# ltdoanh2004/MotionDiffusion-MoE

Hardware: AMD Instinct MI355X
Metric: denoising-steps/sec (B=32, T=196, 263-d, 8 experts) (higher is better)
Workload: dtype bf16

## Files before the change

### motiondiffusion-moe_amd/csrc/rowwise.hip

```cpp
#include "kernels.h"
#include "row.h"

namespace mdm {
extern int g_bf16_variant;
namespace {

template <int NE, bool VEC, int FMT>
__device__ __forceinline__ void ln_chain_rows(const float* __restrict__ x, bool x_h, int64_t M, int D, const float* w1,
                                              const float* b1, void* y1, int y1_h, const float* w2, const float* b2,
                                              void* y2, int y2_h) {
  const int lane = threadIdx.x & 63;
  Row<NE, VEC> ww1, bb1, ww2, bb2;
  ww1.load(w1, D, lane), bb1.load(b1, D, lane);
  if (w2) ww2.load(w2, D, lane), bb2.load(b2, D, lane);
  for (int64_t row = 2 * (blockIdx.x * (int64_t)WPB + (threadIdx.x >> 6)); row < M; row += 2 * (int64_t)gridDim.x * WPB) {
    const bool two = row + 1 < M;
    Row<NE, VEC> r, q;
    if (x_h) {
      r.template load_h16<FMT>((const uint16_t*)x + row * D, D, lane);
      q.template load_h16<FMT>((const uint16_t*)x + (two ? row + 1 : row) * D, D, lane);
    } else {
      r.load(x + row * D, D, lane);
      q.load(x + (two ? row + 1 : row) * D, D, lane);
    }
    r.layernorm(ww1, bb1, D, lane);
    q.layernorm(ww1, bb1, D, lane);
    if (y1) {
      r.template store_mode<FMT>(y1, row, D, lane, y1_h);
      if (two) q.template store_mode<FMT>(y1, row + 1, D, lane, y1_h);
    }
    if (w2) {
      r.layernorm(ww2, bb2, D, lane);
      q.layernorm(ww2, bb2, D, lane);
      r.template store_mode<FMT>(y2, row, D, lane, y2_h);
      if (two) q.template store_mode<FMT>(y2, row + 1, D, lane, y2_h);
    }
  }
}
template <int NE, bool VEC>
__global__ __launch_bounds__(256) void ln_chain_kernel(const float* __restrict__ x, int x_bf, int64_t M, int D,
                                                       const float* w1, const float* b1, void* y1, int y1_bf,
                                                       const float* w2, const float* b2, void* y2, int y2_bf) {
  const int m1 = y1_bf == 4 ? 2 : (y1_bf != 0), m2 = y2_bf == 4 ? 2 : (y2_bf != 0);
  if (((x_bf | y1_bf | y2_bf) & 3) == 2) {
    ln_chain_rows<NE, VEC, 2>(x, x_bf != 0, M, D, w1, b1, y1, m1, w2, b2, y2, m2);
  } else {
    ln_chain_rows<NE, VEC, 1>(x, x_bf != 0, M, D, w1, b1, y1, m1, w2, b2, y2, m2);
  }
}

template <int NE, bool VEC, int FMT>
__device__ __forceinline__ void style_in_rows(const float* __restrict__ x, int64_t M, int D, int S, const float* pw,
                                              const float* pb, const float* sw, const float* sb,
                                              const float* __restrict__ sc, const int* __restrict__ pos4, bool x_h,
                                              void* __restrict__ out, bool out_h) {
  const int lane = threadIdx.x & 63;
  Row<NE, VEC> pww, pbb, sww, sbb;
  if (pw) pww.load(pw, D, lane), pbb.load(pb, D, lane);
  sww.load(sw, D, lane), sbb.load(sb, D, lane);
  for (int64_t row = blockIdx.x * (int64_t)WPB + (threadIdx.x >> 6); row < M; row += (int64_t)gridDim.x * WPB) {
    const float* scb = sc + (row / S) * 2 * (int64_t)D;
    Row<NE, VEC> r, scale, shift;
    scale.load(scb, D, lane);
    shift.load(scb + D, D, lane);
    if (pos4) {
      const int p0 = pos4[row * 4 + 0], p1 = pos4[row * 4 + 1], p2 = pos4[row * 4 + 2], p3 = pos4[row * 4 + 3];
      Row<NE, VEC> a, b, c, d;
      if (x_h) {
        const uint16_t* xh = (const uint16_t*)x;
        a.template load_h16<FMT>(xh + (int64_t)p0 * D, D, lane);
        b.template load_h16<FMT>(xh + (int64_t)p1 * D, D, lane);
        c.template load_h16<FMT>(xh + (int64_t)p2 * D, D, lane);
        d.template load_h16<FMT>(xh + (int64_t)p3 * D, D, lane);
      } else {
        a.load(x + (int64_t)p0 * D, D, lane);
        b.load(x + (int64_t)p1 * D, D, lane);
        c.load(x + (int64_t)p2 * D, D, lane);
        d.load(x + (int64_t)p3 * D, D, lane);
      }
#pragma unroll
      for (int j = 0; j < NE; ++j) r.e[j] = ((a.e[j] + b.e[j]) + (c.e[j] + d.e[j])) * 0.5f;
    } else {
      if (x_h) {
        r.template load_h16<FMT>((const uint16_t*)x + row * D, D, lane);
      } else {
        r.load(x + row * D, D, lane);
      }
    }
    if (pw) {
      r.layernorm(pww, pbb, D, lane);
      float s = 0.f;
#pragma unroll
      for (int j = 0; j < NE; ++j) s += r.e[j] * r.e[j];
      const float inv = sqrtf((float)D) / fmaxf(sqrtf(wave_sum(s)), 1e-12f);
#pragma unroll
      for (int j = 0; j < NE; ++j) r.e[j] *= inv;
    }
    r.layernorm(sww, sbb, D, lane);
#pragma unroll
    for (int j = 0; j < NE; ++j) r.e[j] = silu(r.e[j] * (1.f + scale.e[j]) + shift.e[j]);
    r.template store_to<FMT>(out, row, D, lane, out_h);
  }
}
template <int NE, bool VEC>
__global__ __launch_bounds__(256) void style_in_kernel(const float* __restrict__ x, int64_t M, int D, int S,
                                                       const float* pw, const float* pb,
                                                       const float* sw, const float* sb,
                                                       const float* __restrict__ sc,
                                                       const int* __restrict__ pos4,
                                                       int x_bf,
                                                       void* __restrict__ out, int out_bf) {
  if ((x_bf | out_bf) == 2) {
    style_in_rows<NE, VEC, 2>(x, M, D, S, pw, pb, sw, sb, sc, pos4, x_bf != 0, out, out_bf != 0);
  } else {
    style_in_rows<NE, VEC, 1>(x, M, D, S, pw, pb, sw, sb, sc, pos4, x_bf != 0, out, out_bf != 0);
  }
}

template <int NE, bool VEC>
__global__ __launch_bounds__(256) void moe_gate_kernel(const float* __restrict__ x, int64_t M, int D, int E,
                                                       MoeGateParams p) {
  __shared__ int s_hist[32];
  __shared__ float s_usage[32], s_imp[32];
  if (threadIdx.x < 32) s_hist[threadIdx.x] = 0, s_usage[threadIdx.x] = 0.f, s_imp[threadIdx.x] = 0.f;
  __syncthreads();
  const int lane = threadIdx.x & 63;
  for (int64_t row = blockIdx.x * (int64_t)WPB + (threadIdx.x >> 6); row < M; row += (int64_t)gridDim.x * WPB) {
    Row<NE, VEC> xr;
    xr.load(x + row * D, D, lane);
#pragma unroll
    for (int br = 0; br < 2; ++br) {
      Row<NE, VEC> r = xr;
      r.layernorm(p.ln_w[br], p.ln_b[br], D, lane);
      r.store_as(p.hn, (int64_t)br * M + row, D, lane, p.hn_bf16);
      float logit[16];
      float mx = -INFINITY;
#pragma unroll
      for (int e = 0; e < 16; ++e) {
        logit[e] = -INFINITY;
        if (e < E) {
          Row<NE, VEC> g;
          g.load(p.gate_w[br] + (int64_t)e * D, D, lane);
          float s = 0.f;
#pragma unroll
          for (int j = 0; j < NE; ++j) s += r.e[j] * g.e[j];
          logit[e] = wave_sum(s) + p.gate_b[br][e];
          mx = fmaxf(mx, logit[e]);
        }
      }
      float den = 0.f;
#pragma unroll
      for (int e = 0; e < 16; ++e) {
        logit[e] = e < E ? expf(logit[e] - mx) : 0.f;
        den += logit[e];
      }
      int i1 = 0, i2 = 1;
      float v1 = -1.f, v2 = -1.f;
      if (p.forced_idx) {
        i1 = min(max(p.forced_idx[((int64_t)br * M + row) * 2 + 0], 0), E - 1);
        i2 = min(max(p.forced_idx[((int64_t)br * M + row) * 2 + 1], 0), E - 1);
        v1 = v2 = 0.f;
#pragma unroll
        for (int e = 0; e < 16; ++e) {
          const float pe = logit[e] / den;
          v1 = e == i1 ? pe : v1;
          v2 = e == i2 ? pe : v2;
        }
      } else {
#pragma unroll
        for (int e = 0; e < 16; ++e) {
          const float pe = logit[e] / den;
          if (e < E) {
            if (pe > v1) {
              v2 = v1, i2 = i1;
              v1 = pe, i1 = e;
            } else if (pe > v2) {
              v2 = pe, i2 = e;
            }
          }
        }
        if (!(v2 >= 0.f)) {
          i2 = i1 == 0 ? 1 : 0;
          v1 = v2 = __int_as_float(0x7fc00000);
        }
      }
      if (lane == 0) {
        const int64_t o = ((int64_t)br * M + row) * 2;
        p.top_idx[o] = i1, p.top_idx[o + 1] = i2;
        p.top_val[o] = v1, p.top_val[o + 1] = v2;
        atomicAdd(&s_hist[br * E + i1], 1);
        atomicAdd(&s_hist[br * E + i2], 1);
        atomicAdd(&s_usage[br * E + i1], 1.f);
        atomicAdd(&s_imp[br * E + i1], v1);
        atomicAdd(&s_imp[br * E + i2], v2);
      }
    }
  }
  __syncthreads();
  if (threadIdx.x < 2 * E) {
    const int g = threadIdx.x;
    p.hist[blockIdx.x * 32 + g] = s_hist[g];
    p.uimp[blockIdx.x * 64 + g] = s_usage[g];
    p.uimp[blockIdx.x * 64 + 32 + g] = s_imp[g];
  }
}

template <int NV, bool FAST, int EX = 0, int HNF = -1>
__global__ __launch_bounds__(256) void moe_gate16_kernel(const float* __restrict__ x, int64_t M, int D_rt, int E_rt,
                                                         MoeGateParams p) {
  const int E = EX > 0 ? EX : E_rt;
  const int hnf = HNF >= 0 ? HNF : p.hn_bf16;
  constexpr int D = 64 * NV;
  extern __shared__ __attribute__((aligned(16))) float gsm[];
  float* gw = gsm;
  float* lnw = gsm + 2 * E * D;
  float* lnb = lnw + 2 * D;
  int* s_hist = (int*)(lnb + 2 * D);
  float* s_usage = (float*)(s_hist + 32);
  float* s_imp = s_usage + 32;
  const int l16 = threadIdx.x & 15;
  const int64_t tpb = 16;
  const int64_t stride = (int64_t)gridDim.x * tpb;
  auto load_x = [&](int64_t base, f32x4(&r)[NV]) {
    const int64_t row = base + (threadIdx.x >> 4);
    const int64_t rc = row < M ? row : M - 1;
#pragma unroll
    for (int c = 0; c < NV; ++c) r[c] = *(const f32x4*)(x + rc * D + 4 * (l16 + 16 * c));
  };
  f32x4 vn[NV];
  if constexpr (NV <= 8)
    if (blockIdx.x * tpb < M) load_x(blockIdx.x * tpb, vn);
#pragma unroll
  for (int br = 0; br < 2; ++br) {
    const float* src = p.gate_w[br];
    const int n4 = E * D / 4;
    for (int i0 = threadIdx.x; i0 < n4; i0 += 4 * 256) {
      f32x4 t[4];
#pragma unroll
      for (int j = 0; j < 4; ++j)
        if (i0 + 256 * j < n4) t[j] = *(const f32x4*)(src + 4 * (i0 + 256 * j));
#pragma unroll
      for (int j = 0; j < 4; ++j)
        if (i0 + 256 * j < n4) *(f32x4*)(gw + br * E * D + 4 * (i0 + 256 * j)) = t[j];
    }
  }
  for (int i = threadIdx.x; i < D / 4; i += 256) {
    const f32x4 w0 = *(const f32x4*)(p.ln_w[0] + 4 * i), w1 = *(const f32x4*)(p.ln_w[1] + 4 * i);
    const f32x4 b0 = *(const f32x4*)(p.ln_b[0] + 4 * i), b1 = *(const f32x4*)(p.ln_b[1] + 4 * i);
    *(f32x4*)(lnw + 4 * i) = w0, *(f32x4*)(lnw + D + 4 * i) = w1;
    *(f32x4*)(lnb + 4 * i) = b0, *(f32x4*)(lnb + D + 4 * i) = b1;
  }
  if (threadIdx.x < 32) s_hist[threadIdx.x] = 0, s_usage[threadIdx.x] = 0.f, s_imp[threadIdx.x] = 0.f;
  __syncthreads();
  for (int64_t base = blockIdx.x * tpb; base < M; base += stride) {
    const int64_t row = base + (threadIdx.x >> 4);
    const bool ok = row < M;
    const int64_t rc = ok ? row : M - 1;
    if constexpr (NV > 8) load_x(base, vn);
    f32x4 v[NV];
    float s = 0.f;
#pragma unroll
    for (int c = 0; c < NV; ++c) {
      v[c] = vn[c];
      s += v[c][0] + v[c][1] + v[c][2] + v[c][3];
    }
    if constexpr (NV <= 8)
      if (base + stride < M) load_x(base + stride, vn);
    const float mean = group_sum<16>(s) / D;
    float q = 0.f;
#pragma unroll
    for (int c = 0; c < NV; ++c) {
      v[c] = (f32x4){v[c][0] - mean, v[c][1] - mean, v[c][2] - mean, v[c][3] - mean};
      q += v[c][0] * v[c][0] + v[c][1] * v[c][1] + v[c][2] * v[c][2] + v[c][3] * v[c][3];
    }
    const float rstd = rsqrtf(group_sum<16>(q) / D + 1e-5f);
#pragma unroll
    for (int br = 0; br < 2; ++br) {
      float logit[16];
#pragma unroll
      for (int e = 0; e < 16; ++e) logit[e] = 0.f;
      float amax = 0.f;
#pragma unroll
      for (int c = 0; c < NV; ++c) {
        const int k = 4 * (l16 + 16 * c);
        const f32x4 w = *(const f32x4*)(lnw + br * D + k), b = *(const f32x4*)(lnb + br * D + k);
        const f32x4 h = {v[c][0] * rstd * w[0] + b[0], v[c][1] * rstd * w[1] + b[1], v[c][2] * rstd * w[2] + b[2],
                         v[c][3] * rstd * w[3] + b[3]};
        amax = fmaxf(amax, fmaxf(fmaxf(fabsf(h[0]), fabsf(h[1])), fmaxf(fabsf(h[2]), fabsf(h[3]))));
        if constexpr (HNF >= 0) {
          if constexpr (HNF == 1 || HNF == 2) {
            *(uint2*)((uint16_t*)p.hn + ((int64_t)br * M + rc) * D + k) = make_uint2(pack_h16(HNF, h[0], h[1]), pack_h16(HNF, h[2], h[3]));
          } else if constexpr (HNF == 0) {
            *(f32x4*)((float*)p.hn + ((int64_t)br * M + rc) * D + k) = h;
          } else if constexpr (HNF == 4) {
            static_assert(D % 32 == 0, "lane pairs of store_x2_4p hold k and k ^ 4 of one 32-column block");
            store_x2_4p((uint16_t*)p.hn + ((int64_t)br * M + rc) * 2 * D, k, h[0], h[1], h[2], h[3]);
          }
        } else if (ok && p.hn_bf16 != 3) {
          if (p.hn_bf16 == 4) {
            store_x2_4((uint16_t*)p.hn + ((int64_t)br * M + row) * 2 * D, k, h[0], h[1], h[2], h[3]);
          } else if (p.hn_bf16 == 2) {
            *(uint2*)((uint16_t*)p.hn + ((int64_t)br * M + row) * D + k) = make_uint2(pack_h16(2, h[0], h[1]), pack_h16(2, h[2], h[3]));
          } else if (p.hn_bf16) {
            *(uint2*)((uint16_t*)p.hn + ((int64_t)br * M + row) * D + k) = make_uint2(pack_h16(1, h[0], h[1]), pack_h16(1, h[2], h[3]));
          } else {
            *(f32x4*)((float*)p.hn + ((int64_t)br * M + row) * D + k) = h;
          }
        }
#pragma unroll
        for (int e = 0; e < 16; ++e)
          if (e < E) {
            const f32x4 g = *(const f32x4*)(gw + (br * E + e) * D + k);
            if constexpr (FAST) {
              logit[e] = __builtin_fmaf(h[3], g[3], __builtin_fmaf(h[2], g[2], __builtin_fmaf(h[1], g[1], __builtin_fmaf(h[0], g[0], logit[e]))));
            } else {
              logit[e] += h[0] * g[0] + h[1] * g[1] + h[2] * g[2] + h[3] * g[3];
            }
          }
        if constexpr (EX > 0 && HNF >= 0) __builtin_amdgcn_sched_barrier(0);
      }
      if (hnf == 3) {
        amax = group_max<16>(amax);
        const float scale = amax > 0.f ? amax * (1.f / 448.f) : 1.f, inv = 1.f / scale;
#pragma unroll
        for (int c = 0; c < NV; ++c) {
          const int k = 4 * (l16 + 16 * c);
          const f32x4 w = *(const f32x4*)(lnw + br * D + k), b = *(const f32x4*)(lnb + br * D + k);
          uint32_t q = 0;
          q = __builtin_amdgcn_cvt_pk_fp8_f32((v[c][0] * rstd * w[0] + b[0]) * inv, (v[c][1] * rstd * w[1] + b[1]) * inv, q, false);
          q = __builtin_amdgcn_cvt_pk_fp8_f32((v[c][2] * rstd * w[2] + b[2]) * inv, (v[c][3] * rstd * w[3] + b[3]) * inv, q, true);
          if (HNF >= 0 || ok) *(uint32_t*)((uint8_t*)p.hn + ((int64_t)br * M + (HNF >= 0 ? rc : row)) * D + k) = q;
        }
        if (ok && l16 == 0) p.hn_scale[(int64_t)br * M + row] = scale;
      }
      float mx = -INFINITY, mine = -INFINITY;
#pragma unroll
      for (int e = 0; e < 16; ++e) {
        if (e < E) {
          logit[e] = group_sum<16>(logit[e]) + p.gate_b[br][e];
          mx = fmaxf(mx, logit[e]);
          mine = (l16 == e) ? logit[e] : mine;
        }
      }
      const float den = group_sum<16>(l16 < E ? expf(mine - mx) : 0.f);
      int i1 = 0, i2 = 1;
      float l1 = -INFINITY, l2 = -INFINITY;
      if (p.forced_idx) {
        i1 = min(max(p.forced_idx[((int64_t)br * M + rc) * 2 + 0], 0), E - 1);
        i2 = min(max(p.forced_idx[((int64_t)br * M + rc) * 2 + 1], 0), E - 1);
#pragma unroll
        for (int e = 0; e < 16; ++e) {
          l1 = e == i1 ? logit[e] : l1;
          l2 = e == i2 ? logit[e] : l2;
        }
      } else {
#pragma unroll
        for (int e = 0; e < 16; ++e) {
          if (e < E) {
            if (logit[e] > l1) {
              l2 = l1, i2 = i1;
              l1 = logit[e], i1 = e;
            } else if (logit[e] > l2) {
              l2 = logit[e], i2 = e;
            }
          }
        }
        if (i2 == i1) i2 = i1 == 0 ? 1 : 0;
      }
      const float v1 = expf(l1 - mx) / den, v2 = expf(l2 - mx) / den;
      if (ok && l16 == 0) {
        const int64_t o = ((int64_t)br * M + row) * 2;
        p.top_idx[o] = i1, p.top_idx[o + 1] = i2;
        p.top_val[o] = v1, p.top_val[o + 1] = v2;
        atomicAdd(&s_hist[br * E + i1], 1);
        atomicAdd(&s_hist[br * E + i2], 1);
        atomicAdd(&s_usage[br * E + i1], 1.f);
        atomicAdd(&s_imp[br * E + i1], v1);
        atomicAdd(&s_imp[br * E + i2], v2);
      }
    }
  }
  __syncthreads();
  if (threadIdx.x < 2 * E) {
    const int g = threadIdx.x;
    p.hist[blockIdx.x * 32 + g] = s_hist[g];
    p.uimp[blockIdx.x * 64 + g] = s_usage[g];
    p.uimp[blockIdx.x * 64 + 32 + g] = s_imp[g];
  }
}

__global__ __launch_bounds__(1024) void moe_offsets_kernel(const int* __restrict__ hist_part,
                                                            const float* __restrict__ uimp_part, int nparts, int E,
                                                            int* __restrict__ goff, int* __restrict__ cursor,
                                                            MoeGateParams p) {
  __shared__ int sh[32][33];
  __shared__ float su[32][33], si[32][33];
  __shared__ int tot[32];
  const int g = threadIdx.x & 31, c = threadIdx.x >> 5, G = 2 * E;
  int h = 0;
  float u = 0.f, im = 0.f;
  if (g < G) {
#pragma unroll 4
    for (int b = c; b < nparts; b += 32) {
      h += hist_part[b * 32 + g];
      u += uimp_part[b * 64 + g];
      im += uimp_part[b * 64 + 32 + g];
    }
  }
  sh[c][g] = h, su[c][g] = u, si[c][g] = im;
  __syncthreads();
  if (threadIdx.x < G) {
    int ht = 0;
    float ut = 0.f, it = 0.f;
    for (int k = 0; k < 32; ++k) ht += sh[k][g], ut += su[k][g], it += si[k][g];
    tot[g] = ht;
    cursor[g] = 0;
    const int br = g / E, e = g - br * E;
    if (p.usage[br]) {
      atomicAdd(&p.usage[br][e], ut);
      atomicAdd(&p.importance[br][e], it);
    }
  }
  __syncthreads();
  if (threadIdx.x == 0) {
    int s = 0;
    for (int i = 0; i < G; ++i) {
      goff[i] = s;
      s += tot[i];
    }
    goff[G] = s;
  }
}

__global__ __launch_bounds__(256) void moe_assign_kernel(const int* __restrict__ top_idx, const float* __restrict__ top_val,
                                                         int64_t M, int E, const int* __restrict__ goff,
                                                         int* __restrict__ cursor, int* __restrict__ perm,
                                                         float* __restrict__ rowscale, int* __restrict__ pos4) {
  __shared__ int s_cnt[32], s_base[32];
  const int64_t total = 2 * M * 2;
  for (int64_t base = blockIdx.x * (int64_t)blockDim.x; base < total; base += (int64_t)gridDim.x * blockDim.x) {
    if (threadIdx.x < 32) s_cnt[threadIdx.x] = 0;
    __syncthreads();
    const int64_t i = base + threadIdx.x;
    int g = -1, rank = 0;
    int64_t br = 0, tok = 0;
    int k = 0;
    if (i < total) {
      br = i / (2 * M);
      const int64_t rem = i - br * 2 * M;
      tok = rem >> 1, k = (int)(rem & 1);
      g = (int)br * E + min(max(top_idx[i], 0), E - 1);
      rank = atomicAdd(&s_cnt[g], 1);
    }
    __syncthreads();
    if (threadIdx.x < 2 * E && s_cnt[threadIdx.x]) s_base[threadIdx.x] = atomicAdd(&cursor[threadIdx.x], s_cnt[threadIdx.x]);
    __syncthreads();
    if (g >= 0) {
      const int pos = goff[g] + s_base[g] + rank;
      perm[pos] = (int)(br * M + tok);
      rowscale[pos] = top_val[i];
      pos4[tok * 4 + br * 2 + k] = pos;
    }
    __syncthreads();
  }
}

template <int G>
__device__ __forceinline__ void head_ln(f32x4& v, const float* w, const float* b, int dh, int gl) {
  const float mean = group_sum<G>(v[0] + v[1] + v[2] + v[3]) / dh;
  const f32x4 d = {v[0] - mean, v[1] - mean, v[2] - mean, v[3] - mean};
  const float rstd = rsqrtf(group_sum<G>(d[0] * d[0] + d[1] * d[1] + d[2] * d[2] + d[3] * d[3]) / dh + 1e-5f);
  const f32x4 ww = *(const f32x4*)(w + 4 * gl), bb = *(const f32x4*)(b + 4 * gl);
  v = (f32x4){d[0] * rstd * ww[0] + bb[0], d[1] * rstd * ww[1] + bb[1], d[2] * rstd * ww[2] + bb[2],
              d[3] * rstd * ww[3] + bb[3]};
}

template <int G>
__global__ __launch_bounds__(256) void head_norm_kernel(float* __restrict__ qkv, int64_t units, int H, int dh,
                                                        const float* w, const float* b) {
  const int gl = threadIdx.x % G;
  const int64_t gid = (blockIdx.x * (int64_t)blockDim.x + threadIdx.x) / G;
  const int64_t ng = (int64_t)gridDim.x * blockDim.x / G;
  for (int64_t u = gid; u < units; u += ng) {
    float* p = qkv + u * dh + 4 * gl;
    f32x4 v = *(const f32x4*)p;
    head_ln<G>(v, w, b, dh, gl);
    const int which = (int)((u / H) % 3);
    if (which < 2) {
      const float n = sqrtf(group_sum<G>(v[0] * v[0] + v[1] * v[1] + v[2] * v[2] + v[3] * v[3]));
      const float inv = 1.f / fmaxf(n, 1e-12f);
      v *= inv;
    }
    *(f32x4*)p = v;
  }
}

template <int G>
__global__ __launch_bounds__(256) void den_ln_kernel(const float* __restrict__ num, const float* __restrict__ phi,
                                                     int64_t M, int H, int dh, const float* w, const float* b,
                                                     void* __restrict__ out, int out_bf) {
  const int gl = threadIdx.x % G;
  const int64_t gid = (blockIdx.x * (int64_t)blockDim.x + threadIdx.x) / G;
  const int64_t ng = (int64_t)gridDim.x * blockDim.x / G;
  for (int64_t u = gid; u < M * H; u += ng) {
    const int64_t tok = u / H, h = u - tok * H;
    const f32x4 qf = *(const f32x4*)(phi + (tok * 2 * H + h) * dh + 4 * gl);
    const f32x4 kf = *(const f32x4*)(phi + (tok * 2 * H + H + h) * dh + 4 * gl);
    float den = group_sum<G>(qf[0] * kf[0] + qf[1] * kf[1] + qf[2] * kf[2] + qf[3] * kf[3]);
    den = fmaxf(den, 1e-6f);
    f32x4 v = *(const f32x4*)(num + u * dh + 4 * gl);
    v = (f32x4){v[0] / den, v[1] / den, v[2] / den, v[3] / den};
    head_ln<G>(v, w, b, dh, gl);
    if (out_bf) {
      *(uint2*)((uint16_t*)out + u * dh + 4 * gl) = make_uint2(pack_h16(out_bf, v[0], v[1]), pack_h16(out_bf, v[2], v[3]));
    } else {
      *(f32x4*)((float*)out + u * dh + 4 * gl) = v;
    }
  }
}

template <int G>
__global__ __launch_bounds__(256) void head_softmax_kernel(float* __restrict__ q, int64_t units, int dh) {
  const int gl = threadIdx.x % G;
  const int64_t gid = (blockIdx.x * (int64_t)blockDim.x + threadIdx.x) / G;
  const int64_t ng = (int64_t)gridDim.x * blockDim.x / G;
  for (int64_t u = gid; u < units; u += ng) {
    float* p = q + u * dh + 4 * gl;
    f32x4 v = *(const f32x4*)p;
    const float mx = group_max<G>(fmaxf(fmaxf(v[0], v[1]), fmaxf(v[2], v[3])));
    v = (f32x4){expf(v[0] - mx), expf(v[1] - mx), expf(v[2] - mx), expf(v[3] - mx)};
    const float s = group_sum<G>(v[0] + v[1] + v[2] + v[3]);
    *(f32x4*)p = (f32x4){v[0] / s, v[1] / s, v[2] / s, v[3] / s};
  }
}

#define MDM_HEAD_DISPATCH(dh, CALL)                 \
  do {                                              \
    switch (dh) {                                   \
      case 16: CALL(4); break;                      \
      case 32: CALL(8); break;                      \
      case 64: CALL(16); break;                     \
      case 128: CALL(32); break;                    \
      case 256: CALL(64); break;                    \
      default: return MDM_ERR_UNSUPPORTED;          \
    }                                               \
  } while (0)

__global__ __launch_bounds__(256) void row_softmax_kernel(float* __restrict__ s, int64_t rows, int N, const int32_t* __restrict__ ntok,
                                                          int64_t rows_per_b) {
  const int gl = threadIdx.x & 31;
  const int64_t gid = (blockIdx.x * (int64_t)blockDim.x + threadIdx.x) >> 5;
  const int64_t ng = ((int64_t)gridDim.x * blockDim.x) >> 5;
  for (int64_t r = gid; r < rows; r += ng) {
    float* p = s + r * N;
    const int nv = ntok ? min(max(ntok[r / rows_per_b], 1), N) : N;
    float v[4], mx = -INFINITY;
#pragma unroll
    for (int j = 0; j < 4; ++j) {
      const int i = gl + 32 * j;
      v[j] = i < nv ? p[i] : -INFINITY;
      mx = fmaxf(mx, v[j]);
    }
    mx = group_max<32>(mx);
    float sum = 0.f;
#pragma unroll
    for (int j = 0; j < 4; ++j) {
      v[j] = (gl + 32 * j < nv) ? expf(v[j] - mx) : 0.f;
      sum += v[j];
    }
    sum = group_sum<32>(sum);
#pragma unroll
    for (int j = 0; j < 4; ++j)
      if (gl + 32 * j < N) p[gl + 32 * j] = v[j] / sum;
  }
}

__global__ void col_softmax_kernel(float* __restrict__ k, int B, int N, int D, const int32_t* __restrict__ ntok) {
  const int64_t i = blockIdx.x * (int64_t)blockDim.x + threadIdx.x;
  if (i >= (int64_t)B * D) return;
  const int64_t b = i / D, c = i - b * D;
  float* p = k + b * N * (int64_t)D + c;
  const int nv = ntok ? min(max(ntok[b], 1), N) : N;
  float mx = -INFINITY;
  for (int n = 0; n < nv; ++n) mx = fmaxf(mx, p[(int64_t)n * D]);
  float s = 0.f;
  for (int n = 0; n < nv; ++n) s += expf(p[(int64_t)n * D] - mx);
  for (int n = 0; n < nv; ++n) p[(int64_t)n * D] = expf(p[(int64_t)n * D] - mx) / s;
  for (int n = nv; n < N; ++n) p[(int64_t)n * D] = 0.f;
}

__global__ void sd_fold_mask_cb_kernel(float* __restrict__ cb, int B, int np, int hpp, int N, const int32_t* __restrict__ ntok) {
  const int i = blockIdx.x * blockDim.x + threadIdx.x;
  if (i >= B * np * 128) return;
  const int b = i / (np * 128), col = i & 127;
  if (col < hpp * N && col % N >= min(max(ntok[b], 1), N)) cb[i] = -1e30f;
}

__global__ void sinusoid_kernel(const int64_t* __restrict__ t, int B, int D, float* __restrict__ out) {
  const int i = blockIdx.x * blockDim.x + threadIdx.x;
  const int half = D / 2;
  if (i >= B * D) return;
  const int b = i / D, c = i - b * D;
  float v = 0.f;
  if (c < 2 * half) {
    const int f = c < half ? c : c - half;
    const float freq = expf(-9.210340371976184f * (float)f / (float)half);
    const float arg = (float)t[b] * freq;
    v = c < half ? cosf(arg) : sinf(arg);
  }
  out[i] = v;
}

__global__ void gated_mix_kernel(const float* __restrict__ t, const float* __restrict__ x, int64_t n,
                                 float* __restrict__ out) {
  const int64_t i = blockIdx.x * (int64_t)blockDim.x + threadIdx.x;
  if (i >= n) return;
  const float tv = t[i], xv = x[i];
  const float g = 1.f / (1.f + expf(-(tv + xv)));
  out[i] = g * tv + (1.f - g) * xv;
}

__global__ void text_assemble_kernel(const float* __restrict__ pp, const float* __restrict__ ph, int B, int N0, int P, int Dt,
                                     float* __restrict__ xf_out, float* __restrict__ xf_proj) {
  const int i = blockIdx.x * blockDim.x + threadIdx.x;
  if (i >= B * Dt) return;
  const int b = i / Dt, d = i - b * Dt, N = P + N0;
  float* o = xf_out + (int64_t)b * N * Dt + d;
  float s = 0.f;
  for (int n = 0; n < P; ++n) {
    const float v = pp[n * Dt + d];
    o[(int64_t)n * Dt] = v;
    s += v;
  }
  for (int n = 0; n < N0; ++n) {
    const float v = ph[((int64_t)b * N0 + n) * Dt + d];
    o[(int64_t)(P + n) * Dt] = v;
    s += v;
  }
  xf_proj[i] = s / (float)N;
}

__global__ void gated_mix_gather_kernel(const float* __restrict__ table, const int64_t* __restrict__ ts, int steps,
                                        const float* __restrict__ x, int B, int D, float* __restrict__ out,
                                        uint16_t* __restrict__ out16, int fmt) {
  const int i = blockIdx.x * blockDim.x + threadIdx.x;
  if (i >= B * D) return;
  const int b = i / D, c = i - b * D;
  int64_t t = ts[b];
  t = t < 0 ? 0 : (t >= steps ? steps - 1 : t);
  const float tv = table[t * D + c], xv = x[i];
  const float g = 1.f / (1.f + expf(-(tv + xv)));
  const float v = g * tv + (1.f - g) * xv;
  if (out) out[i] = v;
  if (out16) out16[i] = (uint16_t)(pack_h16(fmt, v, 0.f) & 0xffff);
}

__global__ void iota_i64_kernel(int64_t* dst, int64_t n, int64_t start) {
  const int64_t i = blockIdx.x * (int64_t)blockDim.x + threadIdx.x;
  if (i < n) dst[i] = start + i;
}

__global__ void xattn_gate_kernel(const float* __restrict__ gate, const float* __restrict__ ag, int D,
                                  float* __restrict__ out) {
  const int i = blockIdx.x * blockDim.x + threadIdx.x;
  if (i < D) out[i] = (1.f / (1.f + expf(-gate[i]))) * (1.f / (1.f + expf(-ag[0])));
}

__global__ void halve_lengths_kernel(const int* __restrict__ len, int B, int* __restrict__ out) {
  const int i = blockIdx.x * blockDim.x + threadIdx.x;
  if (i < B) out[i] = (int)(((float)len[i]) / 2.f);
}

__global__ void cfg_step_kernel(const float* __restrict__ x, const float* __restrict__ eps_c,
                                const float* __restrict__ eps_u, const float* __restrict__ noise, int64_t n,
                                const float* __restrict__ tab, int ts, const int* __restrict__ t_ptr, int t_imm, float cfg_scale, int clip,
                                float* __restrict__ x_out, float* __restrict__ x0_out) {
  int t = t_ptr ? *t_ptr : t_imm;
  t = min(max(t, 0), ts - 1);
  const float a = tab[TAB_SQRT_RECIP * ts + t], b = tab[TAB_SQRT_RECIPM1 * ts + t];
  const float c1 = tab[TAB_COEF1 * ts + t], c2 = tab[TAB_COEF2 * ts + t];
  const float sd = t == 0 ? 0.f : expf(0.5f * tab[TAB_LOGVAR * ts + t]);
  for (int64_t i = blockIdx.x * (int64_t)blockDim.x + threadIdx.x; i < n; i += (int64_t)gridDim.x * blockDim.x) {
    const float xv = x[i];
    float x0c = a * xv - b * eps_c[i];
    if (clip) x0c = fminf(fmaxf(x0c, -1.f), 1.f);
    float x0 = x0c;
    if (eps_u) {
      float x0u = a * xv - b * eps_u[i];
      if (clip) x0u = fminf(fmaxf(x0u, -1.f), 1.f);
      x0 = x0u + cfg_scale * (x0c - x0u);
    }
    const float mean = c1 * x0 + c2 * xv;
    x_out[i] = mean + (noise ? sd * noise[i] : 0.f);
    if (x0_out) x0_out[i] = x0;
  }
}

__global__ void ddim_step_kernel(const float* __restrict__ x, const float* __restrict__ eps_in,
                                 const float* __restrict__ noise, int64_t n, const float* __restrict__ tab, int ts,
                                 const int* __restrict__ t_ptr, int t_imm, float eta, int clip,
                                 float* __restrict__ x_out, float* __restrict__ x0_out) {
  int t = t_ptr ? *t_ptr : t_imm;
  t = min(max(t, 0), ts - 1);
  const float a = tab[TAB_SQRT_RECIP * ts + t], b = tab[TAB_SQRT_RECIPM1 * ts + t];
  const float ab = tab[TAB_ACP * ts + t], abp = tab[TAB_ACP_PREV * ts + t];
  const float sigma = eta * sqrtf((1.f - abp) / (1.f - ab)) * sqrtf(1.f - ab / abp);
  const float sq_abp = sqrtf(abp), dir = sqrtf(1.f - abp - sigma * sigma);
  const float nz = t == 0 ? 0.f : 1.f;
  for (int64_t i = blockIdx.x * (int64_t)blockDim.x + threadIdx.x; i < n; i += (int64_t)gridDim.x * blockDim.x) {
    const float xv = x[i];
    float x0 = a * xv - b * eps_in[i];
    if (clip) x0 = fminf(fmaxf(x0, -1.f), 1.f);
    const float eps = (a * xv - x0) / b;
    const float mean = x0 * sq_abp + dir * eps;
    x_out[i] = mean + (noise ? nz * sigma * noise[i] : 0.f);
    if (x0_out) x0_out[i] = x0;
  }
}

__global__ void to_bf16_kernel(const float* __restrict__ src, int64_t n4, uint16_t* __restrict__ dst, int fmt) {
  for (int64_t i = blockIdx.x * (int64_t)blockDim.x + threadIdx.x; i < n4; i += (int64_t)gridDim.x * blockDim.x) {
    const f32x4 v = *(const f32x4*)(src + 4 * i);
    *(uint2*)(dst + 4 * i) = make_uint2(pack_h16(fmt, v[0], v[1]), pack_h16(fmt, v[2], v[3]));
  }
}

__global__ void fill_i64_kernel(int64_t* dst, int64_t n, const int* src) {
  const int64_t i = blockIdx.x * (int64_t)blockDim.x + threadIdx.x;
  if (i < n) dst[i] = (int64_t)*src;
}
__global__ void add_i32_kernel(int* dst, int delta) { *dst += delta; }

inline int unit_grid(int64_t units, int G) {
  int64_t per_block = 256 / G;
  int64_t g = (units + per_block - 1) / per_block;
  return (int)(g < 1 ? 1 : (g > 8192 ? 8192 : g));
}

}

int ln_chain(const float* x, int64_t M, int D, const float* w1, const float* b1, void* y1, int y1_bf, const float* w2,
             const float* b2, void* y2, int y2_bf, hipStream_t s, int x_bf) {
  if (M <= 0) return MDM_OK;
  if (!x || !w1 || !b1 || (w2 && (!b2 || !y2)) || (!w2 && !y1)) return MDM_ERR_ARG;
  if ((unsigned)x_bf > 2 || (y1_bf != 4 && (unsigned)y1_bf > 2) || (y2_bf != 4 && (unsigned)y2_bf > 2) || ((x_bf | y1_bf | y2_bf) & 3) == 3)
    return MDM_ERR_ARG;
  if ((y1_bf == 4 || y2_bf == 4) && D != 256 && D != 512 && D != 1024) return MDM_ERR_UNSUPPORTED;
#define CALL(NE, VEC) \
  hipLaunchKernelGGL((ln_chain_kernel<NE, VEC>), dim3(row_grid((M + 1) / 2)), dim3(256), 0, s, x, x_bf, M, D, w1, b1, y1, y1_bf, w2, b2, y2, y2_bf)
  MDM_ROW_DISPATCH(D, CALL);
#undef CALL
  MDM_RETURN_IF_LAUNCH_FAILED();
  return MDM_OK;
}

int style_in(const float* x, int64_t M, int D, int S, const float* pw, const float* pb, const float* sw,
             const float* sb, const float* sc, const int* pos4, int x_bf, void* out, int out_bf, hipStream_t s) {
  if (M <= 0) return MDM_OK;
  if (!x || !sw || !sb || !sc || !out || S <= 0) return MDM_ERR_ARG;
  if ((unsigned)x_bf > 2 || (unsigned)out_bf > 2 || (x_bf | out_bf) == 3 || (pw && !pb)) return MDM_ERR_ARG;
#define CALL(NE, VEC)                                                                                              \
  hipLaunchKernelGGL((style_in_kernel<NE, VEC>), dim3(row_grid(M)), dim3(256), 0, s, x, M, D, S, pw, pb, sw, sb, sc, \
                     pos4, x_bf, out, out_bf)
  MDM_ROW_DISPATCH(D, CALL);
#undef CALL
  MDM_RETURN_IF_LAUNCH_FAILED();
  return MDM_OK;
}

bool gate16_const_wanted(int nv, int E) {
  if (g_bf16_variant == 27) return false;
  return g_bf16_variant == 26 || ((nv == 8 || nv == 16) && (E == 8 || E == 16));
}
template <int NV, int EX, int HNF, bool FAST = true>
bool launch_gate16_const(int grid, int smem, hipStream_t s, const float* x, int64_t M, int D, int E, const MoeGateParams& p) {
  static DevInt attr_done;
  if (smem > 65536 && smem > attr_done) {
    if (hipFuncSetAttribute((const void*)moe_gate16_kernel<NV, FAST, EX, HNF>, hipFuncAttributeMaxDynamicSharedMemorySize, smem) != hipSuccess)
      return false;
    attr_done = smem;
  }
  hipLaunchKernelGGL((moe_gate16_kernel<NV, FAST, EX, HNF>), dim3(grid), dim3(256), smem, s, x, M, D, E, p);
  return true;
}
template <int NV, int EX>
bool gate16_const_fmt(int grid, int smem, hipStream_t s, const float* x, int64_t M, int D, int E, const MoeGateParams& p) {
  switch (p.hn_bf16) {
    case 1: return launch_gate16_const<NV, EX, 1>(grid, smem, s, x, M, D, E, p);
    case 2: return launch_gate16_const<NV, EX, 2>(grid, smem, s, x, M, D, E, p);
    case 0:
      if constexpr (NV == 8 && EX == 8) return launch_gate16_const<NV, EX, 0, false>(grid, smem, s, x, M, D, E, p);
      return false;
    case 4:
      if constexpr (NV == 8 && EX == 8) return launch_gate16_const<NV, EX, 4, false>(grid, smem, s, x, M, D, E, p);
      return false;
    default: return false;
  }
}
bool gate16_const(int nv, int grid, int smem, hipStream_t s, const float* x, int64_t M, int D, int E, const MoeGateParams& p) {
  if (nv == 8 && E == 8) return gate16_const_fmt<8, 8>(grid, smem, s, x, M, D, E, p);
  if (nv == 8 && E == 16) return gate16_const_fmt<8, 16>(grid, smem, s, x, M, D, E, p);
  if (nv == 16 && E == 8) return gate16_const_fmt<16, 8>(grid, smem, s, x, M, D, E, p);
  if (nv == 16 && E == 16) return gate16_const_fmt<16, 16>(grid, smem, s, x, M, D, E, p);
  return false;
}

int moe_route(const float* x, int64_t M, int D, int E, const MoeGateParams& p, int* goff, int* cursor, int* perm,
              float* rowscale, int* pos4, hipStream_t s) {
  if (M <= 0) return MDM_OK;
  if (E < 2 || E > 16 || !x || !p.hn || !p.hist || !p.uimp || !p.top_idx || !p.top_val) return MDM_ERR_ARG;
  int nparts = 0;
  if (D % 64 == 0 && D <= 1024) {
    const int smem = 2 * E * D * 4 + 4 * D * 4 + 3 * 32 * 4;
    int64_t nb = (M + 15) / 16;
    const int grid = (int)(nb > 512 ? 512 : nb);
    nparts = grid;
    static DevInt attr_done;
    if (smem > 65536 && smem > attr_done) {
      const void* fns[4] = {(const void*)moe_gate16_kernel<16, true>, (const void*)moe_gate16_kernel<16, false>,
                            (const void*)moe_gate16_kernel<8, true>, (const void*)moe_gate16_kernel<8, false>};
      for (const void* fn : fns)
        if (hipFuncSetAttribute(fn, hipFuncAttributeMaxDynamicSharedMemorySize, smem) != hipSuccess) return MDM_ERR_LAUNCH;
      attr_done = smem;
    }
#define GATE16(NV)                                                                                            \
  do {                                                                                                        \
    if (gate16_const_wanted(NV, E) && gate16_const(NV, grid, smem, s, x, M, D, E, p)) {                      \
    } else if (p.hn_bf16 && p.hn_bf16 != 4) {                                                                 \
      hipLaunchKernelGGL((moe_gate16_kernel<NV, true>), dim3(grid), dim3(256), smem, s, x, M, D, E, p);       \
    } else {                                                                                                  \
      hipLaunchKernelGGL((moe_gate16_kernel<NV, false>), dim3(grid), dim3(256), smem, s, x, M, D, E, p);      \
    }                                                                                                         \
  } while (0)
    switch (D / 64) {
      case 1: GATE16(1); break;
      case 2: GATE16(2); break;
      case 4: GATE16(4); break;
      case 8: GATE16(8); break;
      case 16: GATE16(16); break;
      default: return MDM_ERR_UNSUPPORTED;
    }
#undef GATE16
  } else {
  const int gate_grid = row_grid(M) > 512 ? 512 : row_grid(M);
  nparts = gate_grid;
#define CALL(NE, VEC) hipLaunchKernelGGL((moe_gate_kernel<NE, VEC>), dim3(gate_grid), dim3(256), 0, s, x, M, D, E, p)
  MDM_ROW_DISPATCH(D, CALL);
#undef CALL
  }
  hipLaunchKernelGGL(moe_offsets_kernel, dim3(1), dim3(1024), 0, s, p.hist, p.uimp, nparts, E, goff, cursor, p);
  const int64_t total = 4 * M;
  int blocks = (int)((total + 255) / 256);
  hipLaunchKernelGGL(moe_assign_kernel, dim3(blocks > 1024 ? 1024 : blocks), dim3(256), 0, s, p.top_idx, p.top_val, M, E,
                     goff, cursor, perm, rowscale, pos4);
  MDM_RETURN_IF_LAUNCH_FAILED();
  return MDM_OK;
}

int head_norm(float* qkv, int64_t M, int H, int dh, const float* w, const float* b, hipStream_t s) {
  if (M <= 0) return MDM_OK;
  const int64_t units = M * 3 * H;
#define CALL(G) hipLaunchKernelGGL((head_norm_kernel<G>), dim3(unit_grid(units, G)), dim3(256), 0, s, qkv, units, H, dh, w, b)
  MDM_HEAD_DISPATCH(dh, CALL);
#undef CALL
  MDM_RETURN_IF_LAUNCH_FAILED();
  return MDM_OK;
}

int den_ln(const float* num, const float* phi, int64_t M, int H, int dh, const float* w, const float* b, void* out,
           int out_bf, hipStream_t s) {
  if (M <= 0) return MDM_OK;
#define CALL(G) \
  hipLaunchKernelGGL((den_ln_kernel<G>), dim3(unit_grid(M * H, G)), dim3(256), 0, s, num, phi, M, H, dh, w, b, out, out_bf)
  MDM_HEAD_DISPATCH(dh, CALL);
#undef CALL
  MDM_RETURN_IF_LAUNCH_FAILED();
  return MDM_OK;
}

int head_softmax(float* q, int64_t units, int dh, hipStream_t s) {
  if (units <= 0) return MDM_OK;
#define CALL(G) hipLaunchKernelGGL((head_softmax_kernel<G>), dim3(unit_grid(units, G)), dim3(256), 0, s, q, units, dh)
  MDM_HEAD_DISPATCH(dh, CALL);
#undef CALL
  MDM_RETURN_IF_LAUNCH_FAILED();
  return MDM_OK;
}

int row_softmax(float* sc, int64_t rows, int N, hipStream_t s, const int32_t* ntok, int64_t rows_per_b) {
  if (rows <= 0) return MDM_OK;
  if (N < 1 || N > 128 || rows_per_b < 1) return MDM_ERR_UNSUPPORTED;
  hipLaunchKernelGGL(row_softmax_kernel, dim3(unit_grid(rows, 32)), dim3(256), 0, s, sc, rows, N, ntok, rows_per_b);
  MDM_RETURN_IF_LAUNCH_FAILED();
  return MDM_OK;
}

int col_softmax(float* k, int B, int N, int D, hipStream_t s, const int32_t* ntok) {
  const int64_t n = (int64_t)B * D;
  if (n <= 0) return MDM_OK;
  hipLaunchKernelGGL(col_softmax_kernel, dim3((unsigned)((n + 255) / 256)), dim3(256), 0, s, k, B, N, D, ntok);
  MDM_RETURN_IF_LAUNCH_FAILED();
  return MDM_OK;
}

int sd_fold_mask_cb(float* cb, int B, int np, int hpp, int N, const int32_t* ntok, hipStream_t s) {
  const int n = B * np * 128;
  if (n <= 0 || !ntok) return MDM_OK;
  if (!cb || N < 1) return MDM_ERR_ARG;
  hipLaunchKernelGGL(sd_fold_mask_cb_kernel, dim3((n + 255) / 256), dim3(256), 0, s, cb, B, np, hpp, N, ntok);
  MDM_RETURN_IF_LAUNCH_FAILED();
  return MDM_OK;
}

int sinusoid(const int64_t* t, int B, int D, float* out, hipStream_t s) {
  hipLaunchKernelGGL(sinusoid_kernel, dim3((B * D + 255) / 256), dim3(256), 0, s, t, B, D, out);
  MDM_RETURN_IF_LAUNCH_FAILED();
  return MDM_OK;
}

int gated_mix(const float* t, const float* x, int64_t n, float* out, hipStream_t s) {
  hipLaunchKernelGGL(gated_mix_kernel, dim3((unsigned)((n + 255) / 256)), dim3(256), 0, s, t, x, n, out);
  MDM_RETURN_IF_LAUNCH_FAILED();
  return MDM_OK;
}

int text_assemble(const float* pp, const float* ph, int B, int N0, int P, int Dt, float* xf_out, float* xf_proj,
                  hipStream_t s) {
  hipLaunchKernelGGL(text_assemble_kernel, dim3((B * Dt + 255) / 256), dim3(256), 0, s, pp, ph, B, N0, P, Dt, xf_out, xf_proj);
  MDM_RETURN_IF_LAUNCH_FAILED();
  return MDM_OK;
}

int gated_mix_gather(const float* table, const int64_t* ts, int steps, const float* x, int B, int D, float* out,
                     uint16_t* out16, int h16, hipStream_t s) {
  hipLaunchKernelGGL(gated_mix_gather_kernel, dim3((B * D + 255) / 256), dim3(256), 0, s, table, ts, steps, x, B, D, out, out16, h16);
  MDM_RETURN_IF_LAUNCH_FAILED();
  return MDM_OK;
}

int iota_i64(int64_t* dst, int64_t n, int64_t start, hipStream_t s) {
  hipLaunchKernelGGL(iota_i64_kernel, dim3((unsigned)((n + 255) / 256)), dim3(256), 0, s, dst, n, start);
  MDM_RETURN_IF_LAUNCH_FAILED();
  return MDM_OK;
}

int xattn_gate(const float* gate, const float* ag, int D, float* out, hipStream_t s) {
  hipLaunchKernelGGL(xattn_gate_kernel, dim3((D + 255) / 256), dim3(256), 0, s, gate, ag, D, out);
  MDM_RETURN_IF_LAUNCH_FAILED();
  return MDM_OK;
}

int halve_lengths(const int* len, int B, int* out, hipStream_t s) {
  hipLaunchKernelGGL(halve_lengths_kernel, dim3((B + 255) / 256), dim3(256), 0, s, len, B, out);
  MDM_RETURN_IF_LAUNCH_FAILED();
  return MDM_OK;
}

int to_bf16(const float* src, int64_t n, uint16_t* dst, int h16, hipStream_t s) {
  if (n <= 0) return MDM_OK;
  if (n & 3) return MDM_ERR_ARG;
  int64_t blocks = (n / 4 + 255) / 256;
  hipLaunchKernelGGL(to_bf16_kernel, dim3((unsigned)(blocks > 4096 ? 4096 : blocks)), dim3(256), 0, s, src, n / 4, dst, h16);
  MDM_RETURN_IF_LAUNCH_FAILED();
  return MDM_OK;
}

int fill_i64(int64_t* dst, int64_t n, const int* src, hipStream_t s) {
  if (n <= 0) return MDM_OK;
  hipLaunchKernelGGL(fill_i64_kernel, dim3((unsigned)((n + 255) / 256)), dim3(256), 0, s, dst, n, src);
  MDM_RETURN_IF_LAUNCH_FAILED();
  return MDM_OK;
}

int add_i32(int* dst, int delta, hipStream_t s) {
  hipLaunchKernelGGL(add_i32_kernel, dim3(1), dim3(1), 0, s, dst, delta);
  MDM_RETURN_IF_LAUNCH_FAILED();
  return MDM_OK;
}

int cfg_step(const float* x, const float* eps_c, const float* eps_u, const float* noise, int64_t n, const float* tab,
             int ts, const int* t_ptr, int t_imm, float cfg_scale, int clip, float* x_out, float* x0_out, hipStream_t s) {
  if (n <= 0) return MDM_OK;
  if (!x || !eps_c || !tab || !x_out) return MDM_ERR_ARG;
  int blocks = (int)((n + 255) / 256);
  hipLaunchKernelGGL(cfg_step_kernel, dim3(blocks > 2048 ? 2048 : blocks), dim3(256), 0, s, x, eps_c, eps_u, noise, n,
                     tab, ts, t_ptr, t_imm, cfg_scale, clip, x_out, x0_out);
  MDM_RETURN_IF_LAUNCH_FAILED();
  return MDM_OK;
}

int ddim_step(const float* x, const float* eps, const float* noise, int64_t n, const float* tab, int ts, const int* t_ptr,
              int t_imm, float eta, int clip, float* x_out, float* x0_out, hipStream_t s) {
  if (n <= 0) return MDM_OK;
  if (!x || !eps || !tab || !x_out) return MDM_ERR_ARG;
  int blocks = (int)((n + 255) / 256);
  hipLaunchKernelGGL(ddim_step_kernel, dim3(blocks > 2048 ? 2048 : blocks), dim3(256), 0, s, x, eps, noise, n, tab, ts,
                     t_ptr, t_imm, eta, clip, x_out, x0_out);
  MDM_RETURN_IF_LAUNCH_FAILED();
  return MDM_OK;
}

}
```

Baseline: 232.8.

## Fuse MoE offsets and assign into one deterministic per-partition placement kernel

Replaces the single-block offsets kernel and the atomic-cursor assign kernel with one multi-block placement kernel. Each block reduces the per-partition histograms itself to get global group offsets and its own prefix base, then places the tokens it gated, using only shared-memory atomics for rank. Block 0 also reduces the usage and importance statistics. This removes a kernel launch and the serial single-block stage, and drops global cursor atomics. In exchange every block redundantly reduces all partition histograms, and correctness depends on the token-to-block mapping matching the gate kernel's partitioning.

Result: no change. 233.2 (median of 6 runs) (+0.2%).

```diff
diff --git a/motiondiffusion-moe_amd/csrc/rowwise.hip b/motiondiffusion-moe_amd/csrc/rowwise.hip
--- a/motiondiffusion-moe_amd/csrc/rowwise.hip
+++ b/motiondiffusion-moe_amd/csrc/rowwise.hip
@@ -465,6 +465,107 @@
   }
 }
 
+constexpr int kPlaceMaxParts = 512;
+__global__ __launch_bounds__(256) void moe_place_kernel(const int* __restrict__ hist_part, const float* __restrict__ uimp_part,
+                                                        int nparts, int E, const int* __restrict__ top_idx,
+                                                        const float* __restrict__ top_val, int64_t M, int* __restrict__ goff,
+                                                        int* __restrict__ perm, float* __restrict__ rowscale,
+                                                        int* __restrict__ pos4, MoeGateParams p) {
+  constexpr int NQ = kPlaceMaxParts / 32;
+  __shared__ int s_tot[32][33], s_bef[32][33];
+  __shared__ float su[32][33], si[32][33];
+  __shared__ int s_off[33], s_base[32], s_own[32], s_cnt[32];
+  const int G = 2 * E, b = blockIdx.x;
+  const int64_t stride = (int64_t)nparts * 16;
+  const int e = threadIdx.x & 63, br = (e >> 1) & 1, k = e & 1;
+  const int64_t tok0 = (int64_t)b * 16 + (threadIdx.x >> 6) * stride + (e >> 2);
+  int ti0 = 0;
+  float tv0 = 0.f;
+  if (tok0 < M) ti0 = top_idx[(int64_t)br * 2 * M + 2 * tok0 + k], tv0 = top_val[(int64_t)br * 2 * M + 2 * tok0 + k];
+  const int c4 = threadIdx.x & 7, ch = threadIdx.x >> 3;
+  int4 h[NQ];
+#pragma unroll
+  for (int i = 0; i < NQ; ++i) {
+    const int q = ch + 32 * i;
+    h[i] = (4 * c4 < G && q < nparts) ? *(const int4*)(hist_part + q * 32 + 4 * c4) : make_int4(0, 0, 0, 0);
+  }
+  const int own = threadIdx.x < G ? hist_part[b * 32 + threadIdx.x] : 0;
+  if (b == 0) {
+    const int g = threadIdx.x & 31, c = threadIdx.x >> 5;
+#pragma unroll
+    for (int jp = 0; jp < 4; jp += 2) {
+      float uu[2][NQ], ii[2][NQ];
+#pragma unroll
+      for (int j = 0; j < 2; ++j)
+#pragma unroll
+        for (int i = 0; i < NQ; ++i) {
+          const int q = c + 8 * (jp + j) + 32 * i, qc = q < nparts ? q : nparts - 1;
+          uu[j][i] = uimp_part[qc * 64 + g], ii[j][i] = uimp_part[qc * 64 + 32 + g];
+        }
+#pragma unroll
+      for (int j = 0; j < 2; ++j) {
+        const int cc = c + 8 * (jp + j);
+        float u = 0.f, im = 0.f;
+#pragma unroll
+        for (int i = 0; i < NQ; ++i) {
+          const bool in = cc + 32 * i < nparts;
+          u += in ? uu[j][i] : 0.f, im += in ? ii[j][i] : 0.f;
+        }
+        su[cc][g] = u, si[cc][g] = im;
+      }
+    }
+  }
+  int4 t = make_int4(0, 0, 0, 0), be = make_int4(0, 0, 0, 0);
+#pragma unroll
+  for (int i = 0; i < NQ; ++i) {
+    t.x += h[i].x, t.y += h[i].y, t.z += h[i].z, t.w += h[i].w;
+    if (ch + 32 * i < b) be.x += h[i].x, be.y += h[i].y, be.z += h[i].z, be.w += h[i].w;
+  }
+  s_tot[ch][4 * c4 + 0] = t.x, s_tot[ch][4 * c4 + 1] = t.y, s_tot[ch][4 * c4 + 2] = t.z, s_tot[ch][4 * c4 + 3] = t.w;
+  s_bef[ch][4 * c4 + 0] = be.x, s_bef[ch][4 * c4 + 1] = be.y, s_bef[ch][4 * c4 + 2] = be.z, s_bef[ch][4 * c4 + 3] = be.w;
+  if (threadIdx.x < 32) s_cnt[threadIdx.x] = 0;
+  __syncthreads();
+  if (threadIdx.x < G) {
+    const int g = threadIdx.x;
+    int tt = 0, bb = 0;
+    for (int q = 0; q < 32; ++q) tt += s_tot[q][g], bb += s_bef[q][g];
+    s_tot[0][g] = tt, s_base[g] = bb, s_own[g] = own;
+    if (b == 0) {
+      float ut = 0.f, it = 0.f;
+      for (int q = 0; q < 32; ++q) ut += su[q][g], it += si[q][g];
+      const int r = g / E, x = g - r * E;
+      if (p.usage[r]) {
+        atomicAdd(&p.usage[r][x], ut);
+        atomicAdd(&p.importance[r][x], it);
+      }
+    }
+  }
+  __syncthreads();
+  if (threadIdx.x == 0) {
+    int sum = 0;
+    for (int i = 0; i < G; ++i) {
+      s_off[i] = sum;
+      sum += s_tot[0][i];
+    }
+    s_off[G] = sum;
+  }
+  __syncthreads();
+  if (b == 0 && threadIdx.x <= G) goff[threadIdx.x] = s_off[threadIdx.x];
+  for (int64_t tok = tok0; tok - (e >> 2) < M; tok += 4 * stride) {
+    if (tok >= M) continue;
+    const int64_t i = (int64_t)br * 2 * M + 2 * tok + k;
+    const bool first = tok == tok0;
+    const int gg = br * E + min(max(first ? ti0 : top_idx[i], 0), E - 1);
+    const int rank = atomicAdd(&s_cnt[gg], 1);
+    if (rank < s_own[gg]) {
+      const int pos = s_off[gg] + s_base[gg] + rank;
+      perm[pos] = (int)(br * M + tok);
+      rowscale[pos] = first ? tv0 : top_val[i];
+      pos4[tok * 4 + br * 2 + k] = pos;
+    }
+  }
+}
+
 template <int G>
 __device__ __forceinline__ void head_ln(f32x4& v, const float* w, const float* b, int dh, int gl) {
   const float mean = group_sum<G>(v[0] + v[1] + v[2] + v[3]) / dh;
@@ -813,7 +914,7 @@
   if (D % 64 == 0 && D <= 1024) {
     const int smem = 2 * E * D * 4 + 4 * D * 4 + 3 * 32 * 4;
     int64_t nb = (M + 15) / 16;
-    const int grid = (int)(nb > 512 ? 512 : nb);
+    const int grid = (int)(nb > kPlaceMaxParts ? kPlaceMaxParts : nb);
     nparts = grid;
     static DevInt attr_done;
     if (smem > 65536 && smem > attr_done) {
@@ -841,6 +942,12 @@
       default: return MDM_ERR_UNSUPPORTED;
     }
 #undef GATE16
+    if (g_bf16_variant != 71) {
+      hipLaunchKernelGGL(moe_place_kernel, dim3(grid), dim3(256), 0, s, p.hist, p.uimp, nparts, E, p.top_idx, p.top_val, M,
+                         goff, perm, rowscale, pos4, p);
+      MDM_RETURN_IF_LAUNCH_FAILED();
+      return MDM_OK;
+    }
   } else {
   const int gate_grid = row_grid(M) > 512 ? 512 : row_grid(M);
   nparts = gate_grid;
```
